# anassinator/pddp

Hardware: AMD Instinct MI355X
Metric: pddp_iterations_per_sec (higher is better)
Workload: dtype f32; 1 GPU; BASELINE.json configs[1]: cartpole n=4 m=1, known-dynamics iLQR, horizon=100, batch=4096 trajectories per GPU, bounds +-10 (eig-clamp + BoxQP branch), 10 line-search alphas; batch_per_gpu=4096, horizon=100, alphas=10, launch_form=10 rounds per launch, rounds_per_launch=10, backward_kernel_variant=0

## Files before the change

### pddp_amd/csrc/line_search_lds.hpp

```cpp
#pragma once

#include <type_traits>
#include "models.hpp"
#include "problem_args.hpp"
#include "accept.hpp"
#include "riccati_n4.hpp"

namespace pddp {

template <typename T>
PDDP_DEV void group_copy(T* dst, const T* src, int count, int l16) {
  constexpr int kDeep = 8;
  for (int o0 = l16; o0 < count; o0 += 16 * kDeep) {
    T tmp[kDeep];
#pragma unroll
    for (int r = 0; r < kDeep; ++r) {
      const int o = o0 + 16 * r;
      tmp[r] = src[o < count ? o : 0];
    }
#pragma unroll
    for (int r = 0; r < kDeep; ++r) {
      const int o = o0 + 16 * r;
      if (o < count) dst[o] = tmp[r];
    }
// ... 2 lines not shown

PDDP_DEV void store4(float* p, float a, float b, float c, float d) {
  *reinterpret_cast<float4*>(p) = make_float4(a, b, c, d);
}
PDDP_DEV void store4(double* p, double a, double b, double c, double d) {
  *reinterpret_cast<double2*>(p) = make_double2(a, b);
  *reinterpret_cast<double2*>(p + 2) = make_double2(c, d);
}

template <typename T, int n, int m>
PDDP_DEV void control_law(const T* z, const T* zr, const T* gr, const T* us,
                          T alpha, const T* umin, const T* umax, T* un) {
#pragma unroll
  for (int r = 0; r < m; ++r) {
    T s = T(0);
#pragma unroll
    for (int c = 0; c < n; ++c)
      s = n4::fma_(z[c] - zr[c], gr[m + r * n + c], s);
    const T du = n4::fma_(alpha, gr[r], s);
    const T v = us[r] + du;
    un[r] = clamp_nan(v, umin[r], umax[r]);
  }
}
PDDP_DEV float control_law_pk(f32x2 za, f32x2 zb, f32x2 zra, f32x2 zrb,
                              f32x2 g01, f32x2 g23, f32x2 g4u, float alpha,
                              float umin, float umax) {
  const f32x2 da = pk_sub(za, zra), db = pk_sub(zb, zrb);
  float s = n4::fma_(da.x, g01.y, 0.0f);
  s = n4::fma_(da.y, g23.x, s);
  s = n4::fma_(db.x, g23.y, s);
  s = n4::fma_(db.y, g4u.x, s);
  const float du = n4::fma_(alpha, g01.x, s);
  return clamp_nan(g4u.y + du, umin, umax);
}

#ifdef PDDP_WG_TIMELINE
__device__ long long g_search_timeline[1024][12];
#define PDDP_TLS(I)                                                           \
  do {                                                                        \
    if ((threadIdx.x & 255) == 0 && blockIdx.x < 1024)                        \
      g_search_timeline[blockIdx.x][(I) + 4 * (threadIdx.x >> 8)] =           \
          wall_clock64();                                                     \
  } while (0)
#define PDDP_TLS_AT(SLOT)                                                     \
  do {                                                                        \
    if (threadIdx.x == 0 && blockIdx.x < 1024)                                \
      g_search_timeline[blockIdx.x][SLOT] = wall_clock64();                   \
  } while (0)
#else
#define PDDP_TLS(I)
#define PDDP_TLS_AT(SLOT)
#endif

template <typename T>
struct PreStaged {
  const T* Zs;
  const T* Us;
  const T* Gs;
  int status;
  T J_opt;
  T* carry_rows = nullptr;
};
template <typename T, int MODEL, bool FUSED, int WPB, int H, unsigned QM,
          bool DENSE, bool PRE = false>
PDDP_DEV void line_search_lds_body(const ProblemT<T> P,
                                   const LineSearchArgs<T> a,
                                   const AcceptArgs<T> c, T* rec, T* Lout,
                                   unsigned char* smem_raw,
                                   const PreStaged<T> pre,
                                   const unsigned tid = threadIdx.x) {
  using D = ModelDims<MODEL>;
  constexpr int n = D::n, m = D::m;
  constexpr int GS = m + m * n;
  static_assert(H == 1 || (H == 2 && FUSED), "");
  static_assert(!DENSE || (FUSED && H == 1), "");
  static_assert(!PRE || (FUSED && H == 2 && !DENSE), "");
  constexpr int GST = PRE ? GS + m : GS;
  constexpr int UST = PRE ? GS + m : m;
  constexpr int kTailRows = DENSE ? 8 : 4;
  constexpr bool kPaired = PRE && MODEL == PDDP_MODEL_CARTPOLE &&
                           std::is_same<T, float>::value && GST == 6 &&
                           QM == kSparseMask<PDDP_MODEL_CARTPOLE>;
  __shared__ int sh_dec[WPB][4][2];
  const int lane = tid & (kWave - 1);
  const int wave_all = tid >> 6;
  const int wave = H == 1 ? wave_all : wave_all % WPB;
  const int hid = H == 1 ? 0 : wave_all / WPB;
  const int grp = lane >> 4, ai = lane & 15;
  const int N = a.N;
  const int per = DENSE ? N * GS : (N + 1) * n + N * m + N * GS;
  T* smem = reinterpret_cast<T*>(smem_raw) + (size_t)wave * 4 * per;
  const int b0 = (blockIdx.x * WPB + wave) * 4;
  PDDP_TLS(0);

  for (int g = 0; g < (PRE ? 0 : 4); ++g) {
    const int bg = b0 + g;
    if (bg >= a.B) break;
    if (H == 2 && (g & 1) != hid) continue;
    if (a.active != nullptr && a.active[bg] == 0) continue;
    T* dst = smem + (size_t)g * per;
    const T* zs = a.Z + (size_t)bg * (N + 1) * n;
    const T* us = a.U + (size_t)bg * N * m;
    const T* gs = a.gains + (size_t)bg * N * GS;
    if constexpr (DENSE) {
      for (int o = lane; o < N * GS; o += kWave) dst[o] = gs[o];
    } else {
      for (int o = lane; o < (N + 1) * n; o += kWave) dst[o] = zs[o];
      for (int o = lane; o < N * m; o += kWave) dst[(N + 1) * n + o] = us[o];
      for (int o = lane; o < N * GS; o += kWave)
        dst[(N + 1) * n + N * m + o] = gs[o];
    }
  }
  if constexpr (!PRE) __syncthreads();
  PDDP_TLS(1);

  const int b = b0 + grp;
  const bool exists = b < a.B;
  const int bc = exists ? b : a.B - 1;
  const bool attempted =
      exists && (a.active == nullptr || a.active[bc] != 0);
  const bool run =
      attempted && ai < a.A &&
      (PRE ? pre.status == 0
           : (a.bwd_status == nullptr || a.bwd_status[bc] == 0));
  if constexpr (!FUSED) {
    if (!run) return;
  }
  const bool bounded = a.u_min != nullptr && a.u_max != nullptr;
  T umin[m], umax[m];
#pragma unroll
  for (int r = 0; r < m; ++r) {
    umin[r] = bounded ? a.u_min[r] : -(T)__builtin_inff();
    umax[r] = bounded ? a.u_max[r] : (T)__builtin_inff();
  }
  const T* Zs = PRE ? pre.Zs
                    : DENSE ? a.Z + (size_t)bc * (N + 1) * n
                            : smem + (size_t)grp * per;
  const T* Us = PRE ? pre.Us
                    : DENSE ? a.U + (size_t)bc * N * m : Zs + (N + 1) * n;
  const T* Gs = PRE ? pre.Gs : DENSE ? smem + (size_t)grp * per : Us + N * m;
  const size_t zstep_c = (size_t)a.A * n, ustep_c = (size_t)a.A * m;
  AcceptIn<T> acc_in = {};
  if constexpr (FUSED) {
    if (attempted && ai == 0) {
      acc_in = accept_load(c, b);
      if constexpr (PRE) {
        acc_in.bstat = pre.status;
        acc_in.J_opt = pre.J_opt;
      }
    }
  }
  T Jmine = T(0);
  const bool nocand = FUSED && n <= 4 && Lout == nullptr && rec != nullptr &&
                      a.drop_candidates != 0 && N + 1 <= 16 * H * kTailRows;
  const bool store_uc = !(FUSED && n <= 6 && Lout == nullptr &&
                          rec != nullptr && N + 1 <= 16 * H * kTailRows);
  auto rollout = [&](T alpha, T* Zci, size_t zstep, T* Uci, size_t ustep,
                     auto cost) {
    if constexpr (kPaired) {
      typedef float V4_ __attribute__((ext_vector_type(4)));
      V4_ z4 = {Zs[0], Zs[1], Zs[2], Zs[3]};
      float J = 0.0f;
      auto step = [&](const int t) {
        const V4_ zr = *reinterpret_cast<const V4_*>(
            __builtin_assume_aligned(Zs + t * 4, 16));
        const f32x2* g2 = reinterpret_cast<const f32x2*>(
            __builtin_assume_aligned(Gs + t * 6, 8));
        const f32x2 g01 = g2[0], g23 = g2[1], g4u = g2[2];
        const f32x2 sc = sincos_pk(z4.z);
        __builtin_amdgcn_sched_barrier(0);
        __builtin_amdgcn_s_waitcnt(0xC07F);
        const float u = control_law_pk(z4.xy, z4.zw, zr.xy, zr.zw, g01, g23,
                                       g4u, alpha, umin[0], umax[0]);
#pragma unroll
        for (int j = 0; j < 4; ++j) Zci[(size_t)t * zstep + j] = z4[j];
        J += cartpole_cost_pk(P, z4.xy, sc, u);
        if constexpr (decltype(cost)::value) asm("" : "+v"(J));
        f32x2 na, nb;
        cartpole_dynamics_pk(P, z4.xy, z4.zw, sc, u, na, nb);
        z4 = V4_{na.x, na.y, nb.x, nb.y};
      };
      int t = 0;
      for (; t + 3 < N; t += 4) {
        step(t);
        step(t + 1);
        step(t + 2);
        step(t + 3);
      }
#pragma unroll 1
      for (; t < N; ++t) step(t);
      T z[n] = {z4.x, z4.y, z4.z, z4.w};
#pragma unroll
      for (int j = 0; j < n; ++j) Zci[(size_t)N * zstep + j] = z[j];
      const T lf =
          cost_value<T, MODEL>(P, z, nullptr, trig_of<T, MODEL>(z), true);
      return J + lf;
    }
    T z[n], zn[n], un[m];
#pragma unroll
    for (int j = 0; j < n; ++j) z[j] = Zs[j];
    T J = T(0);
    auto step = [&](const int t) {
      T zr[n], gr[GS], us[m];
      if constexpr (PRE && n == 4) {
        typedef T V4_ __attribute__((ext_vector_type(4)));
        const V4_ v = *reinterpret_cast<const V4_*>(
            __builtin_assume_aligned(Zs + t * 4, 16));
        zr[0] = v[0]; zr[1] = v[1]; zr[2] = v[2]; zr[3] = v[3];
      } else {
#pragma unroll
        for (int j = 0; j < n; ++j) zr[j] = Zs[t * n + j];
      }
      if constexpr (PRE && GST == 6) {
        typedef T V2_ __attribute__((ext_vector_type(2)));
        const V2_* g2 = reinterpret_cast<const V2_*>(
            __builtin_assume_aligned(Gs + t * 6, 8));
        const V2_ a0 = g2[0], a1 = g2[1], a2 = g2[2];
        gr[0] = a0[0]; gr[1] = a0[1]; gr[2] = a1[0]; gr[3] = a1[1];
        gr[4] = a2[0]; us[0] = a2[1];
      } else {
#pragma unroll
        for (int j = 0; j < GS; ++j) gr[j] = Gs[t * GST + j];
#pragma unroll
        for (int j = 0; j < m; ++j) us[j] = Us[t * UST + j];
      }
      const Trig<T, MODEL> tr = trig_of<T, MODEL>(z);
      __builtin_amdgcn_sched_barrier(0);
      if constexpr (PRE) __builtin_amdgcn_s_waitcnt(0xC07F);
      control_law<T, n, m>(z, zr, gr, us, alpha, umin, umax, un);
#pragma unroll
      for (int j = 0; j < n; ++j) Zci[(size_t)t * zstep + j] = z[j];
      if constexpr (!PRE) {
        if (store_uc) {
#pragma unroll
          for (int j = 0; j < m; ++j) Uci[(size_t)t * ustep + j] = un[j];
        }
      }
      J += cost_value<T, MODEL, QM>(P, z, un, tr, false);
      dynamics<T, MODEL, false>(P, z, un, tr, zn, nullptr, nullptr);
#pragma unroll
      for (int j = 0; j < n; ++j) z[j] = zn[j];
    };
    int t = 0;
    if constexpr (n <= 4) {
      for (; t + 3 < N; t += 4) {
        step(t);
        step(t + 1);
        step(t + 2);
        step(t + 3);
      }
    }
#pragma unroll 1
    for (; t < N; ++t) step(t);
#pragma unroll
    for (int j = 0; j < n; ++j) Zci[(size_t)N * zstep + j] = z[j];
    const T lf =
        cost_value<T, MODEL>(P, z, nullptr, trig_of<T, MODEL>(z), true);
    return J + lf;
  };
  if (run && hid == 0) {
    const T alpha = a.alphas[ai];
    const int idx = b * a.A + ai;
    const bool compact0 = FUSED && Lout == nullptr && rec != nullptr &&
                          ai == 0 && n <= 6 && N + 1 <= 16 * H * kTailRows;
    T* Zci = compact0 ? rec + (size_t)b * (N + 1) * n
                      : a.Zc + ((size_t)b * (N + 1) * a.A + ai) * n;
    T* Uci = a.Uc + ((size_t)b * N * a.A + ai) * m;
    const size_t zstep = compact0 ? (size_t)n : (nocand ? 0 : zstep_c);
    const size_t ustep = nocand ? 0 : ustep_c;
    Jmine = rollout(alpha, Zci, zstep, Uci, ustep, std::true_type{});
    a.Jc[idx] = Jmine;
  }
  PDDP_TLS(2);

  if constexpr (FUSED) {
    constexpr int kNone = 99;
    const T kInf = (T)__builtin_inff();
    const int nan_first =
        n4::group_min((run && Jmine != Jmine) ? ai : kNone);
    T Jf = (run && Jmine == Jmine) ? Jmine : kInf;
    {
      T y = n4::dpp<0x128>(Jf); Jf = y < Jf ? y : Jf;
      y = n4::dpp<0x12C>(Jf); Jf = y < Jf ? y : Jf;
      y = n4::dpp<(2 | (3 << 2) | (0 << 4) | (1 << 6))>(Jf); Jf = y < Jf ? y : Jf;
      y = n4::dpp<(1 | (0 << 2) | (3 << 4) | (2 << 6))>(Jf); Jf = y < Jf ? y : Jf;
    }
    const int min_first = n4::group_min((run && Jmine == Jf) ? ai : kNone);
    const int amin =
        nan_first != kNone ? nan_first : (min_first != kNone ? min_first : 0);
    const T J_new = nan_first != kNone ? (T)__builtin_nanf("") : Jf;

    int amin_out = -1, fresh_i = 0;
    if (attempted && ai == 0 && hid == 0) {
      bool fr;
      amin_out = accept_decide(c, b, acc_in, amin, J_new, fr);
      fresh_i = fr ? 1 : 0;
    }
    amin_out = __shfl(amin_out, lane & 48);
    fresh_i = __shfl(fresh_i, lane & 48);
    PDDP_TLS_AT(8);
    if constexpr (n <= 4) {
      if (nocand && hid == 0 && __any(amin_out > 0)) {
        if (amin_out > 0 && ai == amin_out)
          rollout(a.alphas[ai], rec + (size_t)b * (N + 1) * n, (size_t)n,
                  a.Uc + ((size_t)b * N * a.A + ai) * m, 0, std::false_type{});
      }
    }
    if constexpr (H == 1) {
      if (!__any(amin_out >= 0)) return;
      __builtin_amdgcn_fence(__ATOMIC_ACQ_REL, "workgroup");
    } else {
      if (hid == 0 && ai == 0) {
        sh_dec[wave][grp][0] = amin_out;
        sh_dec[wave][grp][1] = fresh_i;
      }
      __builtin_amdgcn_fence(__ATOMIC_ACQ_REL, "workgroup");
      __syncthreads();
      amin_out = sh_dec[wave][grp][0];
      fresh_i = sh_dec[wave][grp][1];
    }
    PDDP_TLS_AT(9);
    if (amin_out >= 0) {
      constexpr RecLayout lay(n, m);
      constexpr int S = lay.stride;
      const T* srcz = a.Zc + ((size_t)b * (N + 1) * a.A + amin_out) * n;
      const T* srcu = a.Uc + ((size_t)b * N * a.A + amin_out) * m;
      T* Zb = c.Z + (size_t)b * (N + 1) * n;
      T* Ub = c.U + (size_t)b * N * m;
      T* rec_b = rec + (size_t)b * (N + 1) * S;
      T* Ls = PRE ? nullptr : smem + (size_t)grp * per;
      const T* G = c.gains + (size_t)b * N * GS;
      T* Ga = c.gains_acc + (size_t)b * N * GS;
      T zc[n], uc[m];
      const int t_first = ai + 16 * hid;
      constexpr int KR = kTailRows;
      if (n <= 6 && Lout == nullptr && N + 1 <= 16 * H * KR) {
        T zz[KR][n], uu[KR][m];
        const bool from_rec = rec != nullptr && (amin_out == 0 || nocand);
        const T* cz = from_rec ? rec + (size_t)b * (N + 1) * n : srcz;
        const size_t czs = from_rec ? (size_t)n : zstep_c;
#pragma unroll
        for (int k = 0; k < KR; ++k) {
          const int t = t_first + 16 * H * k;
          const int tz = t <= N ? t : N;
#pragma unroll
          for (int j = 0; j < n; ++j) zz[k][j] = cz[(size_t)tz * czs + j];
        }
        const T* Gl = Gs;
        if constexpr (PRE) {
          for (int t = ai + 16 * hid; t < N; t += 16 * H) {
#pragma unroll
            for (int j = 0; j < GS; ++j) Ga[t * GS + j] = Gl[t * GST + j];
          }
        } else {
          constexpr int kDeep = 8;
          int o = ai + 16 * hid;
          for (; o + 16 * H * (kDeep - 1) < N * GS; o += 16 * H * kDeep) {
            T tmp[kDeep];
#pragma unroll
            for (int r = 0; r < kDeep; ++r) tmp[r] = Gl[o + 16 * H * r];
#pragma unroll
            for (int r = 0; r < kDeep; ++r) Ga[o + 16 * H * r] = tmp[r];
          }
          for (; o < N * GS; o += 16 * H) Ga[o] = Gl[o];
        }
        PDDP_TLS_AT(10);
        const T alpha_w = a.alphas[amin_out];
#pragma unroll
        for (int k = 0; k < KR; ++k) {
          const int t = t_first + 16 * H * k;
          const int tu = t < N ? t : 0;
          if constexpr (kPaired) {
            typedef float V4_ __attribute__((ext_vector_type(4)));
            const V4_ zr = *reinterpret_cast<const V4_*>(
                __builtin_assume_aligned(Zs + tu * 4, 16));
            const f32x2* g2 = reinterpret_cast<const f32x2*>(
                __builtin_assume_aligned(Gs + tu * 6, 8));
            uu[k][0] = control_law_pk(f32x2{zz[k][0], zz[k][1]},
                                      f32x2{zz[k][2], zz[k][3]}, zr.xy, zr.zw,
                                      g2[0], g2[1], g2[2], alpha_w, umin[0],
                                      umax[0]);
            continue;
          }
          T zr[n], gr[GS], us[m];
#pragma unroll
          for (int j = 0; j < n; ++j) zr[j] = Zs[tu * n + j];
#pragma unroll
          for (int j = 0; j < GS; ++j) gr[j] = Gs[tu * GST + j];
#pragma unroll
          for (int j = 0; j < m; ++j) us[j] = Us[tu * UST + j];
          control_law<T, n, m>(zz[k], zr, gr, us, alpha_w, umin, umax, uu[k]);
        }
#pragma unroll
        for (int k = 0; k < KR; ++k) {
          const int t = t_first + 16 * H * k;
          if (t <= N) {
#pragma unroll
            for (int j = 0; j < n; ++j) Zb[t * n + j] = zz[k][j];
          }
          if (t < N) {
#pragma unroll
            for (int j = 0; j < m; ++j) Ub[t * m + j] = uu[k][j];
          }
          if constexpr (PRE) {
            if (pre.carry_rows != nullptr && t <= N && N - t <= 16) {
              T* cr = pre.carry_rows + (N - t) * (n + m);
#pragma unroll
              for (int j = 0; j < n; ++j) cr[j] = zz[k][j];
              if (t < N) {
#pragma unroll
                for (int j = 0; j < m; ++j) cr[n + j] = uu[k][j];
              }
            }
          }
        }
      } else {
      {
        const int tz = t_first <= N ? t_first : N;
        const int tu = t_first < N ? t_first : 0;
#pragma unroll
        for (int j = 0; j < n; ++j) zc[j] = srcz[(size_t)tz * zstep_c + j];
#pragma unroll
        for (int j = 0; j < m; ++j) uc[j] = srcu[(size_t)tu * ustep_c + j];
      }
#pragma unroll 1
      for (int t = t_first; t <= N; t += 16 * H) {
        T zn_[n], un_[m];
        {
          const int t2 = t + 16 * H;
          const int tz = t2 <= N ? t2 : N, tu = t2 < N ? t2 : 0;
#pragma unroll
          for (int j = 0; j < n; ++j) zn_[j] = srcz[(size_t)tz * zstep_c + j];
#pragma unroll
          for (int j = 0; j < m; ++j) un_[j] = srcu[(size_t)tu * ustep_c + j];
        }
        const bool terminal = (t == N);
        T un[m];
#pragma unroll
        for (int j = 0; j < m; ++j) un[j] = terminal ? T(0) : uc[j];
#pragma unroll
        for (int j = 0; j < n; ++j) Zb[t * n + j] = zc[j];
        if (!terminal) {
#pragma unroll
          for (int j = 0; j < m; ++j) Ub[t * m + j] = un[j];
        }
        if (fresh_i && Lout != nullptr) {
          T w[S];
          const T l = record_of<T, MODEL>(P, zc, un, terminal, bounded, a.u_min,
                                         a.u_max, w);
          T* dst = rec_b + (size_t)t * S;
#pragma unroll
          for (int j = 0; j < S; j += 4)
            store4(dst + j, w[j], w[j + 1], w[j + 2], w[j + 3]);
          Lout[(size_t)b * (N + 1) + t] = l;
          Ls[t] = l;
        }
#pragma unroll
        for (int j = 0; j < n; ++j) zc[j] = zn_[j];
// ... 57 lines not shown
```

### pddp_amd/csrc/models.hpp

```cpp
#pragma once

#include <type_traits>
#include "pddp_common.hpp"

namespace pddp {

template <typename T>
struct ProblemT {
  int model, encoding, n, m, na;
  T dt;
  T p[PDDP_MAX_PARAMS - 1];
  T Q[PDDP_MAX_AUG * PDDP_MAX_AUG];
  T Qt[PDDP_MAX_AUG * PDDP_MAX_AUG];
  T R[PDDP_MAX_ACTION * PDDP_MAX_ACTION];
  T goal[PDDP_MAX_AUG];
  T ugoal[PDDP_MAX_ACTION];
};

template <typename T>
inline ProblemT<T> convert_problem(const pddp_problem& s) {
  ProblemT<T> d;
  d.model = s.model;
  d.encoding = s.encoding;
  d.n = s.encoded_size;
// ... 301 lines not shown
    const T nt1d = t1d + sol[1][0] * dt;
    const T nt2d = t2d + sol[2][0] * dt;
    zn[0] = x + nxd * dt;
    zn[1] = nxd;
    zn[2] = t1 + nt1d * dt;
    zn[3] = nt1d;
    zn[4] = t2 + nt2d * dt;
    zn[5] = nt2d;
    if constexpr (JAC) {
      const T da2 = T(2) * l1 * t1d, da3 = T(2) * a1 * t2d;
      const T q0 = sol[0][0], q1 = sol[1][0], q2 = sol[2][0];
      T R[3][6];
      R[0][0] = T(-2) * mu; R[1][0] = T(0); R[2][0] = T(0);
      R[0][1] = -a0 * a2 * c1 - (a0 * l1 * s1 * q1);
      R[1][1] = T(3) * a0 * g * c1 - T(3) * a3 * cd -
                (T(3) * a0 * s1 * q0 - T(3) * a1 * sd * q2);
      R[2][1] = T(3) * a2 * cd - (T(-3) * l1 * sd * q1);
      R[0][2] = -a0 * da2 * s1; R[1][2] = T(0); R[2][2] = T(3) * da2 * sd;
      R[0][3] = -a3 * c2 - (a1 * s2 * q2);
      R[1][3] = T(3) * a3 * cd - (T(3) * a1 * sd * q2);
      R[2][3] = T(-3) * a2 * cd + T(3) * g * c2 -
                (T(3) * s2 * q0 + T(3) * l1 * sd * q1);
      R[0][4] = -da3 * s2; R[1][4] = T(-3) * da3 * sd; R[2][4] = T(0);
      R[0][5] = T(2); R[1][5] = T(0); R[2][5] = T(0);
      solve3<T, 6>(A, R);
#pragma unroll
      for (int r = 0; r < 3; ++r) {
        const int vrow = 2 * r + 1, prow = 2 * r;
#pragma unroll
        for (int q = 0; q < 5; ++q) Fz[vrow * n + (q + 1)] = R[r][q] * dt;
        Fz[vrow * n + vrow] += T(1);
#pragma unroll
        for (int j = 0; j < 6; ++j) Fz[prow * n + j] = Fz[vrow * n + j] * dt;
        Fz[prow * n + prow] += T(1);
        Fu[vrow] = R[r][5] * dt;
        Fu[prow] = Fu[vrow] * dt;
      }
    }
  } else {
    const T mass = P.p[0], alpha = P.p[1];
    const T fr = T(1) - alpha * dt / mass;
#pragma unroll
    for (int i = 0; i < 4; ++i) {
      zn[i] = z[i] + z[4 + i] * dt;
      T acc = z[4 + i] * fr;
      acc += u[i] * dt / mass;
      zn[4 + i] = z[4 + i] + acc * dt;
      if constexpr (JAC) {
        Fz[i * n + i] = T(1);
        Fz[i * n + 4 + i] = dt;
        Fz[(4 + i) * n + 4 + i] = T(1) + fr * dt;
        Fu[(4 + i) * m + i] = dt / mass * dt;
      }
    }
  }
}

template <typename T, int MODEL>
PDDP_DEV void augment(const T* z, const Trig<T, MODEL>& tr, T* a, T* d) {
  using D = ModelDims<MODEL>;
  int q = 0;
#pragma unroll
  for (int i = 0; i < D::na; ++i) {
    if (D::kind[i] == 0) {
      a[i] = z[D::col[i]];
      d[i] = T(1);
    } else if (D::kind[i] == 1) {
      a[i] = tr.s[q];
      d[i] = tr.c[q];
    } else {
      a[i] = tr.c[q];
      d[i] = -tr.s[q];
      ++q;
    }
  }
}

inline unsigned live_mask(const double* Q, int na) {
  unsigned mask = 0;
  for (int i = 0; i < na; ++i)
    for (int j = 0; j < na; ++j)
      if (Q[i * PDDP_MAX_AUG + j] != 0.0) mask |= (1u << i) | (1u << j);
  return mask;
}
template <int MODEL>
constexpr unsigned kFullMask = (1u << ModelDims<MODEL>::na) - 1u;
template <int MODEL>
constexpr unsigned kSparseMask =
    MODEL == PDDP_MODEL_CARTPOLE ? 0b11001u : kFullMask<MODEL>;

template <typename T, int MODEL, unsigned QM = kFullMask<MODEL>>
PDDP_DEV T cost_value(const ProblemT<T>& P, const T* z, const T* u,
                      const Trig<T, MODEL>& tr, bool terminal) {
  using D = ModelDims<MODEL>;
  constexpr int na = D::na, m = D::m;
  const T* Q = terminal ? P.Qt : P.Q;
  T a[na], d[na], dx[na];
  augment<T, MODEL>(z, tr, a, d);
#pragma unroll
  for (int i = 0; i < na; ++i) dx[i] = a[i] - P.goal[i];
  T cost = T(0);
#pragma unroll
  for (int j = 0; j < na; ++j) {
    if (!((QM >> j) & 1u)) continue;
    T dq = T(0);
#pragma unroll
    for (int i = 0; i < na; ++i)
      if ((QM >> i) & 1u) dq += dx[i] * Q[i * PDDP_MAX_AUG + j];
    cost += dq * dx[j];
  }
  if (!terminal) {
    T du[m];
#pragma unroll
    for (int i = 0; i < m; ++i) du[i] = u[i] - P.ugoal[i];
#pragma unroll
    for (int j = 0; j < m; ++j) {
      T dr = T(0);
#pragma unroll
      for (int i = 0; i < m; ++i) dr += du[i] * P.R[i * PDDP_MAX_ACTION + j];
      cost += dr * du[j];
    }
  }
  return cost;
}

PDDP_DEV float cartpole_cost_pk(const ProblemT<float>& P, f32x2 za, f32x2 sc,
                                float F) {
  constexpr int S = PDDP_MAX_AUG;
  const float* Q = P.Q;
  const float dx0 = za.x - P.goal[0];
  const f32x2 dx34 = sc - f32x2{P.goal[3], P.goal[4]};
  float dq0 = __builtin_fmaf(dx0, Q[0 * S + 0], 0.0f);
  f32x2 dq = pk_fma(splat2(dx0), f32x2{Q[0 * S + 3], Q[0 * S + 4]}, splat2(0.0f));
  dq0 = __builtin_fmaf(dx34.x, Q[3 * S + 0], dq0);
  dq = pk_fma(splat2(dx34.x), f32x2{Q[3 * S + 3], Q[3 * S + 4]}, dq);
  dq0 = __builtin_fmaf(dx34.y, Q[4 * S + 0], dq0);
  dq = pk_fma(splat2(dx34.y), f32x2{Q[4 * S + 3], Q[4 * S + 4]}, dq);
  float cost = __builtin_fmaf(dq0, dx0, 0.0f);
  cost = __builtin_fmaf(dq.x, dx34.x, cost);
  cost = __builtin_fmaf(dq.y, dx34.y, cost);
  const float du = F - P.ugoal[0];
  const float dr = __builtin_fmaf(du, P.R[0], 0.0f);
  return __builtin_fmaf(dr, du, cost);
}
PDDP_DEV void cartpole_dynamics_pk(const ProblemT<float>& P, f32x2 za,
                                   f32x2 zb, f32x2 sc, float F, f32x2& na,
                                   f32x2& nb) {
  const float mc = P.p[0], mp = P.p[1], l = P.p[2], mu = P.p[3], g = P.p[4];
  const float dt = P.dt;
  const float x = za.x, xd = za.y, th = zb.x, thd = zb.y, c = sc.y;
  const float a0 = mp * l * thd * thd * sc.x;
  const f32x2 ga = sc * f32x2{g, 3.0f * mp};
  const float a1 = ga.x;
  const float a2 = __builtin_fmaf(-mu, xd, F);
  const float a3 = __builtin_fmaf(-ga.y, c, 4.0f * (mc + mp));
  const f32x2 m1 = f32x2{mc + mp, 3.0f * mp} * splat2(a1);
  float num_t = __builtin_fmaf(a2, c, m1.x);
  num_t = num_t + num_t;
  num_t = __builtin_fmaf(a0, c, num_t);
  const float ia3 = inv_(a3);
  float num_x = m1.y * c;
  num_x = __builtin_fmaf(2.0f, a0, num_x);
  num_x = __builtin_fmaf(4.0f, a2, num_x);
  const float il = 1.0f / l;
  const f32x2 acc = f32x2{num_x, -3.0f * num_t} * f32x2{ia3, ia3 * il};
  const float nxd = __builtin_fmaf(acc.x, dt, xd);
  const float nthd = __builtin_fmaf(acc.y, dt, thd);
  na = f32x2{__builtin_fmaf(nxd, dt, x), nxd};
  nb = f32x2{__builtin_fmaf(nthd, dt, th), nthd};
}

template <typename T, int MODEL, unsigned QM = kFullMask<MODEL>>
PDDP_DEV T cost_derivs(const ProblemT<T>& P, const T* z, const T* u,
                       const Trig<T, MODEL>& tr, bool terminal, T* l_z,
                       T* l_zz, T* l_u, T* l_uu) {
  using D = ModelDims<MODEL>;
  constexpr int na = D::na, n = D::n, m = D::m;
  const T* Q = terminal ? P.Qt : P.Q;
  T a[na], d[na], dx[na], g[na];
  augment<T, MODEL>(z, tr, a, d);
#pragma unroll
  for (int i = 0; i < na; ++i) dx[i] = a[i] - P.goal[i];
  T cost = T(0);
#pragma unroll
  for (int j = 0; j < na; ++j) {
    if (!((QM >> j) & 1u)) continue;
    T dq = T(0);
#pragma unroll
    for (int i = 0; i < na; ++i)
      if ((QM >> i) & 1u) dq += dx[i] * Q[i * PDDP_MAX_AUG + j];
    cost += dq * dx[j];
  }
#pragma unroll
  for (int i = 0; i < na; ++i) {
    T s = T(0);
    if ((QM >> i) & 1u) {
#pragma unroll
      for (int j = 0; j < na; ++j)
        if ((QM >> j) & 1u)
          s += (Q[i * PDDP_MAX_AUG + j] + Q[j * PDDP_MAX_AUG + i]) * dx[j];
    }
    g[i] = s;
  }
#pragma unroll
  for (int c = 0; c < n; ++c) l_z[c] = T(0);
#pragma unroll
  for (int i = 0; i < na; ++i)
    if ((QM >> i) & 1u) l_z[D::col[i]] += d[i] * g[i];
#pragma unroll
  for (int i = 0; i < n * n; ++i) l_zz[i] = T(0);
#pragma unroll
  for (int i = 0; i < na; ++i) {
    if (!((QM >> i) & 1u)) continue;
#pragma unroll
    for (int k = 0; k < na; ++k)
      if ((QM >> k) & 1u)
        l_zz[D::col[i] * n + D::col[k]] +=
            d[i] *
            ((Q[i * PDDP_MAX_AUG + k] + Q[k * PDDP_MAX_AUG + i]) * d[k]);
  }
#pragma unroll
  for (int i = 0; i < na; ++i)
    if (D::kind[i] != 0 && ((QM >> i) & 1u))
      l_zz[D::col[i] * n + D::col[i]] += g[i] * (-a[i]);
  if (!terminal) {
    T du[m];
#pragma unroll
    for (int i = 0; i < m; ++i) du[i] = u[i] - P.ugoal[i];
#pragma unroll
    for (int j = 0; j < m; ++j) {
      T dr = T(0);
#pragma unroll
      for (int i = 0; i < m; ++i) dr += du[i] * P.R[i * PDDP_MAX_ACTION + j];
      cost += dr * du[j];
    }
#pragma unroll
    for (int i = 0; i < m; ++i) {
      T s = T(0);
#pragma unroll
      for (int j = 0; j < m; ++j) {
        const T rij = P.R[i * PDDP_MAX_ACTION + j] + P.R[j * PDDP_MAX_ACTION + i];
        s += rij * du[j];
        l_uu[i * m + j] = rij;
      }
      l_u[i] = s;
    }
  }
  return cost;
}

template <typename T, int MODEL, unsigned QM = kFullMask<MODEL>>
PDDP_DEV T record_of(const ProblemT<T>& P, const T* z, const T* un,
                     bool terminal, bool bounded, const T* u_min,
                     const T* u_max, T* w) {
  using D = ModelDims<MODEL>;
  constexpr int n = D::n, m = D::m;
  constexpr RecLayout lay(n, m);
  constexpr int S = lay.stride;
  T u[m], zn[n];
  T Fz[n * n], Fu[n * m], lz[n], lzz[n * n], lu[m], luu[m * m];
#pragma unroll
  for (int j = 0; j < m; ++j) {
    u[j] = bounded ? clamp1(un[j], u_min[j], u_max[j]) : un[j];
    lu[j] = T(0);
  }
#pragma unroll
  for (int j = 0; j < m * m; ++j) luu[j] = T(0);
  Trig<T, MODEL> tr = trig_of<T, MODEL>(z);
  if (!terminal) {
    dynamics<T, MODEL, true>(P, z, u, tr, zn, Fz, Fu);
  } else {
#pragma unroll
    for (int j = 0; j < n * n; ++j) Fz[j] = T(0);
#pragma unroll
    for (int j = 0; j < n * m; ++j) Fu[j] = T(0);
  }
  const T l =
      cost_derivs<T, MODEL, QM>(P, z, u, tr, terminal, lz, lzz, lu, luu);
#pragma unroll
  for (int j = 0; j < n * n; ++j) w[lay.oFz + j] = Fz[j];
#pragma unroll
  for (int j = 0; j < n * n; ++j) w[lay.oLzz + j] = lzz[j];
#pragma unroll
  for (int j = 0; j < n * m; ++j) w[lay.oFu + j] = Fu[j];
#pragma unroll
  for (int j = 0; j < m * n; ++j) w[lay.oLuz + j] = T(0);
#pragma unroll
  for (int j = 0; j < n; ++j) w[lay.oLz + j] = lz[j];
#pragma unroll
  for (int j = 0; j < m * m; ++j) w[lay.oLuu + j] = luu[j];
#pragma unroll
  for (int j = 0; j < m; ++j) w[lay.oLu + j] = lu[j];
#pragma unroll
  for (int j = 0; j < m; ++j) w[lay.oU + j] = un[j];
#pragma unroll
  for (int j = lay.oU + m; j < S; ++j) w[j] = T(0);
  return l;
}

}
```

### pddp_amd/csrc/problem_args.hpp

```cpp
#pragma once

#include "pddp_common.hpp"

namespace pddp {

template <typename T>
struct RolloutArgs {
  int B, N;
  const T* z0;
  const T* U;
  const T* u_min;
  const T* u_max;
  const uint8_t* mask;
  T* Z;
};

constexpr int kDerivThreads = 64;

template <typename T>
struct DerivArgs {
  int B, N;
  const T* Z;
  const T* U;
  const T* u_min;
  const T* u_max;
  const uint8_t* mask;
  T* rec;
  T* L;
  T* J;
  int32_t* state;
};

template <typename T>
struct LineSearchArgs {
  int B, N, A;
  const T* Z;
  const T* U;
  const T* gains;
  const T* alphas;
  const T* u_min;
  const T* u_max;
  const uint8_t* active;
  const int32_t* bwd_status;
  T* Zc;
  T* Uc;
  T* Jc;
  int drop_candidates = 0;
};

template <typename T>
inline bool args_ok(const DerivArgs<T>& a) {
  return !(a.B <= 0 || a.N <= 0 || !a.Z || !a.U || !a.rec || !a.L || !a.J);
}
template <typename T>
inline bool args_ok(const LineSearchArgs<T>& a, bool int_lanes) {
  if (a.B <= 0 || a.N <= 0 || a.A <= 0 || !a.Z || !a.U || !a.gains ||
      !a.alphas || !a.Zc || !a.Uc || !a.Jc)
    return false;
  return !(int_lanes && (long long)a.B * a.A > 0x7fffffffLL);
}
template <typename T>
inline dim3 search_lanes(const LineSearchArgs<T>& a) {
  return dim3((unsigned)(((long long)a.B * a.A + kWave - 1) / kWave));
}
template <typename Args, typename Extra>
struct With {
  Args a;
  Extra x;
};

inline int check_problem(const pddp_problem* p) {
  if (p == nullptr) return PDDP_E_BADARG;
  if (p->encoding != PDDP_ENC_IGNORE_UNCERTAINTY) return PDDP_E_UNSUPPORTED;
  switch (p->model) {
    case PDDP_MODEL_CARTPOLE:
    case PDDP_MODEL_DOUBLE_CARTPOLE:
    case PDDP_MODEL_PENDULUM:
    case PDDP_MODEL_RENDEZVOUS:
      return 0;
  }
  return PDDP_E_UNSUPPORTED;
}

#define PDDP_DISPATCH_MODEL(FN, T, p, args, st)                                \
  switch ((p)->model) {                                                        \
    case PDDP_MODEL_CARTPOLE:                                                  \
      return FN<T, PDDP_MODEL_CARTPOLE>(*(p), args, st);                       \
    case PDDP_MODEL_DOUBLE_CARTPOLE:                                           \
      return FN<T, PDDP_MODEL_DOUBLE_CARTPOLE>(*(p), args, st);                \
    case PDDP_MODEL_PENDULUM:                                                  \
      return FN<T, PDDP_MODEL_PENDULUM>(*(p), args, st);                       \
    default:                                                                   \
      return FN<T, PDDP_MODEL_RENDEZVOUS>(*(p), args, st);                     \
  }

}
```

### pddp_amd/csrc/problem_kernels.hip

```cpp
#include <type_traits>
#include "models.hpp"
#include "problem_args.hpp"
#include "model_params.hpp"
#include "accept.hpp"
#include "riccati_n4.hpp"
#include "line_search_lds.hpp"

namespace pddp {


template <typename T, int MODEL>
PDDP_DEV ProblemT<T> problem_of_row(const ProblemT<T>& shared, const T* table,
                                    int b) {
  ProblemT<T> P = shared;
  write_params_and_goals<T, MODEL>(P, table + (size_t)b * PDDP_BATCH_ROW);
  return P;
}


template <typename T, int MODEL>
__global__ __launch_bounds__(kWave) void nominal_rollout_kernel(
    ProblemT<T> P, RolloutArgs<T> a) {
#define PDDP_PROBLEM_OF_B
#include "rollout_body.inc"
// ... 94 lines not shown
  const dim3 lanes = search_lanes(a);
  if (w.x != nullptr) {
    PDDP_LAUNCH((batch_line_search_kernel<T, MODEL>), lanes, dim3(kWave), 0,
                st, P, a, w.x);
    return launch_status();
  }
  using D = ModelDims<MODEL>;
  const size_t per = (size_t)(a.N + 1) * D::n + (size_t)a.N * D::m +
                     (size_t)a.N * (D::m + D::m * D::n);
  const size_t lds = 4 * per * sizeof(T);
  if (a.A <= 16 && lds <= 64 * 1024) {
    if (4 * lds <= 64 * 1024) {
      if (stage_cost_on<MODEL, kSparseMask<MODEL>>(p))
        PDDP_LAUNCH((line_search_lds_kernel<T, MODEL, false, 4, 1,
                                            kSparseMask<MODEL>>),
                           dim3((a.B + 15) / 16), dim3(kWave * 4), 4 * lds, st,
                           P, a, AcceptArgs<T>{}, (T*)nullptr, (T*)nullptr);
      else
        PDDP_LAUNCH((line_search_lds_kernel<T, MODEL, false, 4>),
                           dim3((a.B + 15) / 16), dim3(kWave * 4), 4 * lds, st,
                           P, a, AcceptArgs<T>{}, (T*)nullptr, (T*)nullptr);
    } else
      PDDP_LAUNCH((line_search_lds_kernel<T, MODEL, false, 1>),
                         dim3((a.B + 3) / 4), dim3(kWave), lds, st, P, a,
                         AcceptArgs<T>{}, (T*)nullptr, (T*)nullptr);
    return launch_status();
  }
  PDDP_LAUNCH((line_search_kernel<T, MODEL>), lanes, dim3(kWave), 0, st, P,
              a);
  return launch_status();
}

template <typename T>
struct SearchAcceptArgs {
  LineSearchArgs<T> ls;
  AcceptArgs<T> ac;
  T* rec;
  T* L;
};
inline int& search_form_choice() {
  static int choice = 0;
  return choice;
}
template <typename T, int MODEL>
static int launch_search_accept(const pddp_problem& p, SearchAcceptArgs<T> a,
                                hipStream_t st) {
  const ProblemT<T> P = convert_problem<T>(p);
  using D = ModelDims<MODEL>;
  const size_t per = (size_t)(a.ls.N + 1) * D::n + (size_t)a.ls.N * D::m +
                     (size_t)a.ls.N * (D::m + D::m * D::n);
  const size_t lds = 4 * per * sizeof(T);
  if (a.ls.A > 16 || lds > 64 * 1024) return PDDP_E_UNSUPPORTED;
  a.ac.n = D::n;
  a.ac.m = D::m;
  if constexpr (sizeof(T) == 4 && D::n <= 4) {
    const int mode = search_form_choice();
    const size_t lds_dense =
        16 * (size_t)a.ls.N * (D::m + D::m * D::n) * sizeof(T);
    const bool dense =
        mode == 2 || (mode == 0 && a.ls.B > 8192 && a.ls.B <= 49152);
    if (dense && 4 * lds <= 64 * 1024 && lds_dense <= 40 * 1024 &&
        a.ls.N + 1 <= 128) {
      if (stage_cost_on<MODEL, kSparseMask<MODEL>>(p))
        PDDP_LAUNCH((line_search_lds_kernel<T, MODEL, true, 4, 1,
                                            kSparseMask<MODEL>, true>),
                    dim3((a.ls.B + 15) / 16), dim3(kWave * 4), lds_dense, st,
                    P, a.ls, a.ac, a.rec, a.L);
      else
        PDDP_LAUNCH((line_search_lds_kernel<T, MODEL, true, 4, 1,
                                            kFullMask<MODEL>, true>),
                    dim3((a.ls.B + 15) / 16), dim3(kWave * 4), lds_dense, st,
                    P, a.ls, a.ac, a.rec, a.L);
      return launch_status();
    }
  }
  if (4 * lds <= 64 * 1024) {
    if (stage_cost_on<MODEL, kSparseMask<MODEL>>(p))
      PDDP_LAUNCH((line_search_lds_kernel<T, MODEL, true, 4, 2,
                                          kSparseMask<MODEL>>),
                         dim3((a.ls.B + 15) / 16), dim3(kWave * 8), 4 * lds, st,
                         P, a.ls, a.ac, a.rec, a.L);
    else
      PDDP_LAUNCH((line_search_lds_kernel<T, MODEL, true, 4, 2>),
                         dim3((a.ls.B + 15) / 16), dim3(kWave * 8), 4 * lds, st,
                         P, a.ls, a.ac, a.rec, a.L);
  } else
    PDDP_LAUNCH((line_search_lds_kernel<T, MODEL, true, 1>),
                       dim3((a.ls.B + 3) / 4), dim3(kWave), lds, st, P, a.ls,
                       a.ac, a.rec, a.L);
  return launch_status();
}

template <typename T>
int default_rollout(const pddp_problem& p, RolloutArgs<T> a, hipStream_t st);
template <typename T>
int default_derivs(const pddp_problem& p, DerivArgs<T> a, hipStream_t st);
template <typename T>
int default_line_search(const pddp_problem& p, LineSearchArgs<T> a,
                        hipStream_t st);
static bool is_default_encoding(const pddp_problem* p) {
  return p != nullptr && (p->encoding == PDDP_ENC_UPPER_TRIANGULAR_CHOLESKY ||
                          p->encoding == PDDP_ENC_VARIANCE_ONLY ||
                          p->encoding == PDDP_ENC_STANDARD_DEVIATION_ONLY ||
                          p->encoding == PDDP_ENC_FULL_COVARIANCE_MATRIX);
}


template <typename T>
static int nominal_rollout_impl(const pddp_problem* p, bool batch,
                                const T* table, int B, int N, const T* z0,
                                const T* U, const T* u_min, const T* u_max,
                                const uint8_t* mask, T* Z, void* stream) {
  if (B <= 0 || N <= 0 || (batch && !table) || !z0 || !U || !Z)
    return PDDP_E_BADARG;
  With<RolloutArgs<T>, const T*> w{{B, N, z0, U, u_min, u_max, mask, Z},
                                   table};
  if (!batch && is_default_encoding(p))
    return default_rollout<T>(*p, w.a, (hipStream_t)stream);
  if (int rc = check_problem(p)) return rc;
  PDDP_DISPATCH_MODEL(launch_rollout, T, p, w, (hipStream_t)stream)
}

template <typename T>
static int derivs_impl(const pddp_problem* p, bool batch, const T* table,
                       int B, int N, const T* Z, const T* U, const T* u_min,
                       const T* u_max, const uint8_t* mask, T* rec, T* L, T* J,
                       int32_t* state, void* stream) {
  With<DerivArgs<T>, const T*> w{
      {B, N, Z, U, u_min, u_max, mask, rec, L, J, state}, table};
  if (!args_ok(w.a) || (batch && !table)) return PDDP_E_BADARG;
  if (!batch && is_default_encoding(p))
    return default_derivs<T>(*p, w.a, (hipStream_t)stream);
  if (int rc = check_problem(p)) return rc;
  PDDP_DISPATCH_MODEL(launch_derivs, T, p, w, (hipStream_t)stream)
}

template <typename T>
static int line_search_impl(const pddp_problem* p, bool batch, const T* table,
                            int B, int N, int A, const T* Z, const T* U,
                            const T* gains, const T* alphas, const T* u_min,
                            const T* u_max, const uint8_t* active,
                            const int32_t* bwd_status, T* Zc, T* Uc, T* Jc,
                            void* stream) {
  With<LineSearchArgs<T>, const T*> w{{B, N, A, Z, U, gains, alphas, u_min,
                                       u_max, active, bwd_status, Zc, Uc, Jc},
                                      table};
  if (!args_ok(w.a, batch) || (batch && !table)) return PDDP_E_BADARG;
  if (!batch && is_default_encoding(p))
    return default_line_search<T>(*p, w.a, (hipStream_t)stream);
  if (int rc = check_problem(p)) return rc;
  PDDP_DISPATCH_MODEL(launch_line_search, T, p, w, (hipStream_t)stream)
}

inline int& search_candidates_choice() {
  static int choice = 0;
  return choice;
}

template <typename T>
static int search_accept_impl(const pddp_problem* p, int B, int N, int A, T* Z,
                              T* U, const T* gains, const T* alphas,
                              const T* u_min, const T* u_max, uint8_t* active,
                              const int32_t* bwd_status, T* Zc, T* Uc, T* Jc,
                              double tol, double max_reg, int n_iterations,
                              T* gains_acc, T* J_opt, double* mu,
                              double* delta, int32_t* state, int32_t* iter,
                              uint8_t* fresh, int32_t* n_live, T* rec, T* L,
                              void* stream) {
  if (int rc = check_problem(p)) return rc;
  if (B <= 0 || N <= 0 || A <= 0 || !Z || !U || !gains || !alphas || !active ||
      !bwd_status || !Zc || !Uc || !Jc || !gains_acc || !J_opt || !mu ||
      !delta || !state || !iter || !fresh || (L != nullptr && !rec))
    return PDDP_E_BADARG;
  SearchAcceptArgs<T> a;
  a.ls = LineSearchArgs<T>{B, N, A, Z, U, gains, alphas, u_min, u_max, active,
                           bwd_status, Zc, Uc, Jc};
  a.ac = AcceptArgs<T>{B, N, 0, 0, A, Zc, Uc, Jc, gains, bwd_status, tol,
                       max_reg, n_iterations, Z, U, gains_acc, J_opt, mu, delta,
                       state, iter, active, fresh, n_live};
  a.rec = rec;
  a.L = L;
  const double cand_bytes =
      (double)B * A * ((double)(N + 1) * p->encoded_size +
                       (double)N * p->action_size) * sizeof(T);
  const int mode = search_candidates_choice();
  a.ls.drop_candidates =
      (L == nullptr && rec != nullptr &&
       (mode == 2 || (mode == 0 && cand_bytes > 200e6))) ? 1 : 0;
  PDDP_DISPATCH_MODEL(launch_search_accept, T, p, a, (hipStream_t)stream)
}

}

extern "C" {

#ifdef PDDP_WG_TIMELINE
int pddp_debug_search_timeline(long long* out) {
  hipDeviceSynchronize();
  hipMemcpyFromSymbol(out, HIP_SYMBOL(pddp::g_search_timeline),
                      sizeof(long long) * 1024 * 12);
  return 0;
}
#endif

int pddp_search_form(int mode) {
  const int prev = pddp::search_form_choice();
  if (mode >= 0 && mode <= 2) pddp::search_form_choice() = mode;
  return prev;
}
int pddp_search_candidates(int mode) {
  const int prev = pddp::search_candidates_choice();
  if (mode >= 0 && mode <= 2) pddp::search_candidates_choice() = mode;
  return prev;
}

#define PDDP_PROBLEM_ENTRY_POINTS(SUF, T)                                      \
  int pddp_search_accept_##SUF(                                                \
      const pddp_problem* p, int B, int N, int A, T* Z, T* U, const T* gains,  \
      const T* alphas, const T* u_min, const T* u_max, uint8_t* active,        \
      const int32_t* bwd_status, T* Zc, T* Uc, T* Jc, double tol,              \
      double max_reg, int n_iterations, T* gains_acc, T* J_opt, double* mu,    \
      double* delta, int32_t* state, int32_t* iter, uint8_t* fresh,            \
      int32_t* n_live, T* rec, T* L, void* stream) {                           \
    return pddp::search_accept_impl<T>(                                        \
        p, B, N, A, Z, U, gains, alphas, u_min, u_max, active, bwd_status, Zc, \
        Uc, Jc, tol, max_reg, n_iterations, gains_acc, J_opt, mu, delta,       \
        state, iter, fresh, n_live, rec, L, stream);                           \
  }                                                                            \
  int pddp_nominal_rollout_##SUF(                                              \
      const pddp_problem* p, int B, int N, const T* z0, const T* U,            \
      const T* u_min, const T* u_max, const uint8_t* mask, T* Z,               \
      void* stream) {                                                          \
    return pddp::nominal_rollout_impl<T>(p, false, nullptr, B, N, z0, U,       \
                                         u_min, u_max, mask, Z, stream);       \
  }                                                                            \
  int pddp_derivs_##SUF(const pddp_problem* p, int B, int N, const T* Z,       \
                        const T* U, const T* u_min, const T* u_max,            \
                        const uint8_t* mask, T* rec, T* L, T* J,               \
                        int32_t* state, void* stream) {                        \
    return pddp::derivs_impl<T>(p, false, nullptr, B, N, Z, U, u_min, u_max,   \
                                mask, rec, L, J, state, stream);               \
  }                                                                            \
  int pddp_line_search_##SUF(                                                  \
      const pddp_problem* p, int B, int N, int A, const T* Z, const T* U,      \
      const T* gains, const T* alphas, const T* u_min, const T* u_max,         \
      const uint8_t* active, const int32_t* bwd_status, T* Zc, T* Uc, T* Jc,   \
      void* stream) {                                                          \
    return pddp::line_search_impl<T>(p, false, nullptr, B, N, A, Z, U, gains,  \
                                     alphas, u_min, u_max, active, bwd_status, \
                                     Zc, Uc, Jc, stream);                      \
  }                                                                            \
                 \
  int pddp_nominal_rollout_batch_##SUF(                                        \
      const pddp_problem* p, const T* table, int B, int N, const T* z0,        \
      const T* U, const T* u_min, const T* u_max, const uint8_t* mask, T* Z,   \
      void* stream) {                                                          \
    return pddp::nominal_rollout_impl<T>(p, true, table, B, N, z0, U, u_min,   \
                                         u_max, mask, Z, stream);              \
  }                                                                            \
  int pddp_derivs_batch_##SUF(                                                 \
      const pddp_problem* p, const T* table, int B, int N, const T* Z,         \
      const T* U, const T* u_min, const T* u_max, const uint8_t* mask, T* rec, \
      T* L, T* J, int32_t* state, void* stream) {                              \
    return pddp::derivs_impl<T>(p, true, table, B, N, Z, U, u_min, u_max,      \
                                mask, rec, L, J, state, stream);               \
  }                                                                            \
  int pddp_line_search_batch_##SUF(                                            \
      const pddp_problem* p, const T* table, int B, int N, int A, const T* Z,  \
      const T* U, const T* gains, const T* alphas, const T* u_min,             \
      const T* u_max, const uint8_t* active, const int32_t* bwd_status, T* Zc, \
      T* Uc, T* Jc, void* stream) {                                            \
    return pddp::line_search_impl<T>(p, true, table, B, N, A, Z, U, gains,     \
                                     alphas, u_min, u_max, active, bwd_status, \
                                     Zc, Uc, Jc, stream);                      \
  }

PDDP_PROBLEM_ENTRY_POINTS(f32, float)
PDDP_PROBLEM_ENTRY_POINTS(f64, double)
#undef PDDP_PROBLEM_ENTRY_POINTS

}
```

### pddp_amd/csrc/round_n4.hip

```cpp
#include "round_n4_body.hpp"

namespace pddp {

template <unsigned QM, bool MULTI>
__global__ __launch_bounds__(2 * n4e::kWaves * kWave) void round_n4_kernel(
    RiccatiArgs<float> a, n4d::GenArgs<float> gen, ProblemT<float> prob,
    LineSearchArgs<float> ls, AcceptArgs<float> ac, float* scratch,
    int rounds, long long* phase_ticks, int use_carry) {
  round_n4_body<QM, MULTI, n4e::kBrEigBox>(a, gen, prob, ls, ac, scratch,
                                           rounds, phase_ticks, use_carry);
}

static int launch_round_n4(const pddp_problem& p, const RiccatiArgs<float>& a,
                           const n4d::GenArgs<float>& gen,
                           const LineSearchArgs<float>& ls,
                           const AcceptArgs<float>& ac, float* scratch,
                           int rounds, long long* phase_ticks,
                           hipStream_t st) {
  N4NominalPlan pl;
  if (const int rc = n4_nominal_plan(p, sizeof(float), true, a.B, a.N, ls.A,
                                     a.u_min != nullptr, a.u_max != nullptr,
                                     a.branch, rounds, 0, pl))
    return rc;
  if (pl.br != n4e::kBrEigBox)
    return launch_round_n4_branches(p, pl, a, gen, ls, ac, scratch, rounds,
                                    phase_ticks, st);
#define PDDP_K(QM)                                                            \
  (pl.multi ? round_n4_kernel<QM, true> : round_n4_kernel<QM, false>)
  return launch_dyn_lds(PDDP_N4_BY_MASK(PDDP_K), dim3(pl.grid),
                        dim3(pl.threads), pl.lds, st, a, gen,
                        convert_problem<float>(p), ls, ac, scratch, rounds,
                        phase_ticks, pl.use_carry);
#undef PDDP_K
}

}

extern "C" int pddp_round_nominal_f32(
    const pddp_problem* problem, int B, int N, int A, float* Z, float* U,
    const float* alphas, const float* u_min, const float* u_max, int branch,
    uint8_t* active, uint8_t* fresh, float* gains, int32_t* bwd_status,
    float* L, float* J_opt, float* Zc, float* Uc, float* Jc, double tol,
    double max_reg, int n_iterations, float* gains_acc, double* mu,
    double* delta, int32_t* state, int32_t* iter, int32_t* n_live,
    float* scratch, int rounds, long long* phase_ticks, void* stream) {
  if (problem == nullptr || B <= 0 || N <= 0 || A <= 0 || !Z || !U || !alphas ||
      !active || !fresh || !gains || !bwd_status || !L || !J_opt || !Zc ||
      !Uc || !Jc || !gains_acc || !mu || !delta || !state || !iter || !scratch)
    return PDDP_E_BADARG;
  if (branch != PDDP_BRANCH_EIG && branch != PDDP_BRANCH_CHOLESKY)
    return PDDP_E_BADARG;
  const pddp::NominalArgs<float> sw = pddp::nominal_args<float>(
      *problem, B, N, Z, U, u_min, u_max, mu, branch, active, fresh, gains,
      bwd_status, L, J_opt);
  const pddp::LineSearchArgs<float> ls{B, N, A, Z, U, gains, alphas, u_min,
                                       u_max, active, bwd_status, Zc, Uc, Jc};
  const pddp::AcceptArgs<float> ac{
      B, N, 4, 1, A, Zc, Uc, Jc, gains, bwd_status, tol, max_reg, n_iterations,
      Z, U, gains_acc, J_opt, mu, delta, state, iter, active, fresh, n_live};
  return pddp::launch_round_n4(*problem, sw.a, sw.gen, ls, ac, scratch, rounds,
                               phase_ticks, (hipStream_t)stream);
}

#ifdef PDDP_WG_TIMELINE
extern "C" int pddp_debug_round_timeline(long long* sweep, long long* search) {
  (void)hipDeviceSynchronize();
  (void)hipMemcpyFromSymbol(sweep, HIP_SYMBOL(pddp::n4e::g_elem_timeline),
                            sizeof(long long) * 1024 * 12);
  (void)hipMemcpyFromSymbol(search, HIP_SYMBOL(pddp::g_search_timeline),
                            sizeof(long long) * 1024 * 12);
  return 0;
}
#endif
```

Baseline: 50.27 million trajectory-iterations/s.

## Checkpoint every fourth state in paired rollout and rebuild winner trajectory in parallel

In the fused n4 round kernel, drop_candidates mode can now be switched on through search_candidates_choice. The paired cartpole rollout then writes only every fourth state of each candidate trajectory. When a nonzero alpha wins, the 16 lanes rebuild that trajectory together, each re-simulating one 3-step segment from its checkpoint, instead of one lane redoing the whole rollout. This cuts global stores during the line search at the cost of extra recompute and a fence on acceptance. The feature is gated by a static choice that defaults to 0, so it may be off by default; the diff also reorders one multiply in the cartpole dynamics.

```diff
diff --git a/pddp_amd/csrc/line_search_lds.hpp b/pddp_amd/csrc/line_search_lds.hpp
--- a/pddp_amd/csrc/line_search_lds.hpp
+++ b/pddp_amd/csrc/line_search_lds.hpp
@@ -178,16 +178,20 @@
   }
   T Jmine = T(0);
   const bool nocand = FUSED && n <= 4 && Lout == nullptr && rec != nullptr &&
-                      a.drop_candidates != 0 && N + 1 <= 16 * H * kTailRows;
+                      a.drop_candidates != 0 && N + 1 <= 16 * H * kTailRows &&
+                      (!PRE || kPaired);
   const bool store_uc = !(FUSED && n <= 6 && Lout == nullptr &&
                           rec != nullptr && N + 1 <= 16 * H * kTailRows);
   auto rollout = [&](T alpha, T* Zci, size_t zstep, T* Uci, size_t ustep,
-                     auto cost) {
+                     auto cost, bool ckpt = false) {
     if constexpr (kPaired) {
       typedef float V4_ __attribute__((ext_vector_type(4)));
       V4_ z4 = {Zs[0], Zs[1], Zs[2], Zs[3]};
       float J = 0.0f;
-      auto step = [&](const int t) {
+      const size_t zin = ckpt ? 0 : zstep;
+      const size_t ztrip = 4 * zstep;
+      T* zp = ckpt ? Zci + 3 * zstep : Zci;
+      auto step = [&](const int t, T* const zrow) {
         const V4_ zr = *reinterpret_cast<const V4_*>(
             __builtin_assume_aligned(Zs + t * 4, 16));
         const f32x2* g2 = reinterpret_cast<const f32x2*>(
@@ -199,7 +203,7 @@
         const float u = control_law_pk(z4.xy, z4.zw, zr.xy, zr.zw, g01, g23,
                                        g4u, alpha, umin[0], umax[0]);
 #pragma unroll
-        for (int j = 0; j < 4; ++j) Zci[(size_t)t * zstep + j] = z4[j];
+        for (int j = 0; j < 4; ++j) zrow[j] = z4[j];
         J += cartpole_cost_pk(P, z4.xy, sc, u);
         if constexpr (decltype(cost)::value) asm("" : "+v"(J));
         f32x2 na, nb;
@@ -208,13 +212,16 @@
       };
       int t = 0;
       for (; t + 3 < N; t += 4) {
-        step(t);
-        step(t + 1);
-        step(t + 2);
-        step(t + 3);
+        T* const z1 = zp + zin;
+        T* const z2 = z1 + zin;
+        step(t, zp);
+        step(t + 1, z1);
+        step(t + 2, z2);
+        step(t + 3, z2 + zin);
+        zp += ztrip;
       }
 #pragma unroll 1
-      for (; t < N; ++t) step(t);
+      for (; t < N; ++t) step(t, Zci + (size_t)t * zstep);
       T z[n] = {z4.x, z4.y, z4.z, z4.w};
 #pragma unroll
       for (int j = 0; j < n; ++j) Zci[(size_t)N * zstep + j] = z[j];
@@ -292,9 +299,11 @@
     T* Zci = compact0 ? rec + (size_t)b * (N + 1) * n
                       : a.Zc + ((size_t)b * (N + 1) * a.A + ai) * n;
     T* Uci = a.Uc + ((size_t)b * N * a.A + ai) * m;
-    const size_t zstep = compact0 ? (size_t)n : (nocand ? 0 : zstep_c);
+    const size_t zstep =
+        compact0 ? (size_t)n : (nocand && !PRE ? 0 : zstep_c);
     const size_t ustep = nocand ? 0 : ustep_c;
-    Jmine = rollout(alpha, Zci, zstep, Uci, ustep, std::true_type{});
+    Jmine = rollout(alpha, Zci, zstep, Uci, ustep, std::true_type{},
+                    PRE && nocand && !compact0);
     a.Jc[idx] = Jmine;
   }
   PDDP_TLS(2);
@@ -325,11 +334,54 @@
     amin_out = __shfl(amin_out, lane & 48);
     fresh_i = __shfl(fresh_i, lane & 48);
     PDDP_TLS_AT(8);
-    if constexpr (n <= 4) {
+    if constexpr (n <= 4 && !PRE) {
       if (nocand && hid == 0 && __any(amin_out > 0)) {
         if (amin_out > 0 && ai == amin_out)
           rollout(a.alphas[ai], rec + (size_t)b * (N + 1) * n, (size_t)n,
                   a.Uc + ((size_t)b * N * a.A + ai) * m, 0, std::false_type{});
+      }
+    }
+    if constexpr (kPaired) {
+      if (__builtin_expect(nocand && hid == 0 && __any(amin_out > 0), 0)) {
+        __builtin_amdgcn_fence(__ATOMIC_ACQ_REL, "workgroup");
+        if (amin_out > 0) {
+          typedef float V4_ __attribute__((ext_vector_type(4)));
+          const float alpha_w = a.alphas[amin_out];
+          float* cz = rec + (size_t)b * (N + 1) * n;
+          float* wz = a.Zc + ((size_t)b * (N + 1) * a.A + amin_out) * n;
+          const int trips = N >> 2;
+          for (int k = ai; k < trips; k += 16) {
+            int t = k ? 4 * k - 1 : 0;
+            V4_ z4 = k ? *reinterpret_cast<const V4_*>(wz + t * zstep_c)
+                       : *reinterpret_cast<const V4_*>(
+                             __builtin_assume_aligned(Zs, 16));
+            *reinterpret_cast<V4_*>(cz + t * n) = z4;
+            if (k == 0) *reinterpret_cast<V4_*>(wz) = z4;
+#pragma unroll 1
+            for (int i = 0; i < 3; ++i, ++t) {
+              const V4_ zr = *reinterpret_cast<const V4_*>(
+                  __builtin_assume_aligned(Zs + t * 4, 16));
+              const f32x2* g2 = reinterpret_cast<const f32x2*>(
+                  __builtin_assume_aligned(Gs + t * 6, 8));
+              const f32x2 g01 = g2[0], g23 = g2[1], g4u = g2[2];
+              const f32x2 sc = sincos_pk(z4.z);
+              const float u = control_law_pk(z4.xy, z4.zw, zr.xy, zr.zw, g01,
+                                             g23, g4u, alpha_w, umin[0],
+                                             umax[0]);
+              f32x2 na, nb;
+              cartpole_dynamics_pk(P, z4.xy, z4.zw, sc, u, na, nb);
+              z4 = V4_{na.x, na.y, nb.x, nb.y};
+              if (((t + 1) & 3) != 3) {
+                *reinterpret_cast<V4_*>(cz + (t + 1) * n) = z4;
+                *reinterpret_cast<V4_*>(wz + (t + 1) * zstep_c) = z4;
+              }
+            }
+          }
+          const int t = (trips ? 4 * trips - 1 : 0) + ai;
+          if (t <= N)
+            *reinterpret_cast<V4_*>(cz + t * n) =
+                *reinterpret_cast<const V4_*>(wz + t * zstep_c);
+        }
       }
     }
     if constexpr (H == 1) {
diff --git a/pddp_amd/csrc/models.hpp b/pddp_amd/csrc/models.hpp
--- a/pddp_amd/csrc/models.hpp
+++ b/pddp_amd/csrc/models.hpp
@@ -477,9 +477,9 @@
   const float a0 = mp * l * thd * thd * sc.x;
   const f32x2 ga = sc * f32x2{g, 3.0f * mp};
   const float a1 = ga.x;
+  const f32x2 m1 = f32x2{mc + mp, 3.0f * mp} * splat2(a1);
   const float a2 = __builtin_fmaf(-mu, xd, F);
   const float a3 = __builtin_fmaf(-ga.y, c, 4.0f * (mc + mp));
-  const f32x2 m1 = f32x2{mc + mp, 3.0f * mp} * splat2(a1);
   float num_t = __builtin_fmaf(a2, c, m1.x);
   num_t = num_t + num_t;
   num_t = __builtin_fmaf(a0, c, num_t);
diff --git a/pddp_amd/csrc/problem_args.hpp b/pddp_amd/csrc/problem_args.hpp
--- a/pddp_amd/csrc/problem_args.hpp
+++ b/pddp_amd/csrc/problem_args.hpp
@@ -48,6 +48,11 @@
   int drop_candidates = 0;
 };
 
+inline int& search_candidates_choice() {
+  static int choice = 0;
+  return choice;
+}
+
 template <typename T>
 inline bool args_ok(const DerivArgs<T>& a) {
   return !(a.B <= 0 || a.N <= 0 || !a.Z || !a.U || !a.rec || !a.L || !a.J);
diff --git a/pddp_amd/csrc/problem_kernels.hip b/pddp_amd/csrc/problem_kernels.hip
--- a/pddp_amd/csrc/problem_kernels.hip
+++ b/pddp_amd/csrc/problem_kernels.hip
@@ -270,11 +270,6 @@
   PDDP_DISPATCH_MODEL(launch_line_search, T, p, w, (hipStream_t)stream)
 }
 
-inline int& search_candidates_choice() {
-  static int choice = 0;
-  return choice;
-}
-
 template <typename T>
 static int search_accept_impl(const pddp_problem* p, int B, int N, int A, T* Z,
                               T* U, const T* gains, const T* alphas,
diff --git a/pddp_amd/csrc/round_n4.hip b/pddp_amd/csrc/round_n4.hip
--- a/pddp_amd/csrc/round_n4.hip
+++ b/pddp_amd/csrc/round_n4.hip
@@ -53,8 +53,9 @@
   const pddp::NominalArgs<float> sw = pddp::nominal_args<float>(
       *problem, B, N, Z, U, u_min, u_max, mu, branch, active, fresh, gains,
       bwd_status, L, J_opt);
-  const pddp::LineSearchArgs<float> ls{B, N, A, Z, U, gains, alphas, u_min,
-                                       u_max, active, bwd_status, Zc, Uc, Jc};
+  pddp::LineSearchArgs<float> ls{B, N, A, Z, U, gains, alphas, u_min,
+                                 u_max, active, bwd_status, Zc, Uc, Jc};
+  ls.drop_candidates = pddp::search_candidates_choice() == 2 ? 1 : 0;
   const pddp::AcceptArgs<float> ac{
       B, N, 4, 1, A, Zc, Uc, Jc, gains, bwd_status, tol, max_reg, n_iterations,
       Z, U, gains_acc, J_opt, mu, delta, state, iter, active, fresh, n_live};
```

After: 49.72 million trajectory-iterations/s. -1.1%, worse.
